# Mictronics/readsb-protobuf

Measured on AMD Instinct MI355X. Metric: IQ Msamples/s, 2.4 MSPS UC8, Mode S demodulation (CRC-valid msgs/s alongside), higher is better.
Workload: dtype int32 (u8 IQ -> u16 magnitude -> int32 correlators, 24-bit CRC)

## Files before the change

readsb-protobuf_amd/csrc/msd_kernels.hip:

```cpp
#include <hip/hip_runtime.h>

#include <cstdlib>

#include "msd_internal.h"
#include "msd_dc_chain_asm.h"
#include "msd_kernels.h"

#ifndef MSD_ARENA_NT
#define MSD_ARENA_NT 1
#endif
#if MSD_ARENA_NT
#define MSD_ARENA_STORE(v, p) __builtin_nontemporal_store((v), (p))
#else
#define MSD_ARENA_STORE(v, p) (*(p) = (v))
#endif
typedef uint32_t msd_v4u __attribute__((ext_vector_type(4)));
__device__ __forceinline__ void arena_store16(const uint4 v, uint4 *p)
{
#if MSD_ARENA_NT
    msd_v4u x = {v.x, v.y, v.z, v.w};
    __builtin_nontemporal_store(x, reinterpret_cast<msd_v4u *>(p));
#else
    *p = v;
#endif
}
#ifndef MSD_AC_PRIO
#define MSD_AC_PRIO 2
#endif
#ifndef MSD_SLICER_SIGN
#define MSD_SLICER_SIGN 1
#endif
#ifndef MSD_TESTS_SWZ
#define MSD_TESTS_SWZ 1
#endif
#ifndef MSD_PRIO_CONV
#define MSD_PRIO_CONV 0
#endif
#ifndef MSD_TESTS_PRE_PLANE
#define MSD_TESTS_PRE_PLANE 1
#endif
#ifndef MSD_PRIO_GATHER
#define MSD_PRIO_GATHER MSD_PRIO_CONV
#endif
#ifndef MSD_PRIO_TESTS
#define MSD_PRIO_TESTS 1
#endif
#ifndef MSD_PRIO_CAND
#define MSD_PRIO_CAND 2
#endif
#ifndef MSD_PRIO_STEPB
#define MSD_PRIO_STEPB 3
#endif
#include "msd_emit_impl.h"
#include "msd_pred_impl.h"
#include "msd_mag_impl.h"

#pragma clang fp contract(off)

#ifdef MSD_KERNEL_TIMING
__device__ unsigned long long g_msd_tlast_dummy;
__device__ __forceinline__ uint32_t msd_cycles()
{
    return (uint32_t)__builtin_readcyclecounter();
}
#define TDECL uint32_t tacc_[12] = {0}; uint32_t tlast_ = msd_cycles();
#define TCOARSE(k) (MSD_KERNEL_TIMING + 0 != 2 || (k) == 0 || (k) == 2 || (k) == 9)
#define TMARK(k) if (TCOARSE(k)) { const uint32_t n_ = msd_cycles(); tacc_[k] += n_ - tlast_; tlast_ = n_; }
#define TMARKF(k) if (MSD_KERNEL_TIMING + 0 != 2) { const uint32_t n_ = msd_cycles(); tacc[k] += n_ - *tlast; *tlast = n_; }
#define TFLUSH if (P.timers && (threadIdx.x & 63) == 0) { for (int k_ = 0; k_ < 12; ++k_) atomicAdd(&P.timers[k_], (unsigned long long)tacc_[k_]); }
#else
#define TDECL
#define TMARK(k)
#define TMARKF(k)
#define TFLUSH
#endif

namespace {

constexpr int WAVES = MSD_SCAN_WAVES;
constexpr int NT = MSD_SCAN_THREADS;
constexpr int WT_MAX = MSD_TILE;
constexpr int FRONT = MSD_HALO_FRONT;
__host__ __device__ constexpr int tile_runs(int fmt)
{
    return (fmt == MSD_FMT_SC16 || fmt == MSD_FMT_SC16Q11) ? 1 : WT_MAX / 1024;
}
constexpr int HC = 64;
constexpr int SC = 64;
constexpr int LUT_STRIDE = MSD_LUT_STRIDE;

static_assert(WT_MAX == 1024 || WT_MAX == 2048 || WT_MAX == 4096, "each lane scans one, two or four runs of 16 consecutive positions");
static_assert(WT_MAX <= 8192, "a position inside a tile has 13 bits in the hit and slot words");
static_assert(FRONT % 8 == 0, "whole load groups");
static_assert(MSD_CHUNK_SAMPLES % WT_MAX == 0, "a tile never straddles two buffers");

constexpr int OFF_SYN = 0;
constexpr int OFF_SL = OFF_SYN + MSD_SYNH_WORDS * 4;
constexpr int OFF_WGC = OFF_SL + MSD_SLICER_WORDS * 4;
constexpr int OFF_WAVE = (OFF_WGC + WAVES * 16 + 15) & ~15;
constexpr int W_MAGS = 0;
constexpr int W_HITS = W_MAGS + (FRONT + WT_MAX + 8) * 2;
constexpr int W_TRYL = W_HITS + HC * 4;
constexpr int W_SIDX = W_TRYL + HC * 5 * 2;
constexpr int W_SMETA = W_SIDX + HC * 8 * 2;
constexpr int W_SMSG = W_SMETA + SC * 4;
constexpr int W_SCRC = W_SMSG + SC * 16;
constexpr int W_SRES = W_SCRC + SC * 4;
constexpr int W_SQOFF = W_SRES + SC * 8;
constexpr int W_BYTES = W_SQOFF + SC * 4;
constexpr int OFF_LUT = OFF_WAVE + WAVES * W_BYTES;
constexpr int LDS_COMMON = OFF_LUT;
constexpr int LDS_UC8 = OFF_LUT + (MSD_LUT_GLOBAL ? 0 : 128 * LUT_STRIDE * 2);
static_assert(OFF_WAVE % 16 == 0 && W_SMSG % 16 == 0 && W_BYTES % 16 == 0 && OFF_LUT % 16 == 0 && W_SIDX % 4 == 0,
              "LDS carve offsets must stay aligned");
static_assert(LDS_UC8 <= 160 * 1024, "one workgroup per CU: 160 KiB of LDS");


template <int FMT>
struct RawGroup {
    static constexpr int WORDS = (FMT == MSD_FMT_SC16 || FMT == MSD_FMT_SC16Q11) ? 8 : 4;
    uint32_t w[WORDS];
};

template <int FMT>
__device__ __forceinline__ uint32_t fetch_group(const MsdScanParams &P, int64_t n, RawGroup<FMT> &r)
{
    constexpr int BPS = RawGroup<FMT>::WORDS / 2;
    const int64_t rel = n - (int64_t)P.batch_first;
    const int64_t left = (int64_t)P.nsamples - rel;
    const uint8_t *src = reinterpret_cast<const uint8_t *>(P.lut);
    uint32_t valid = 0;
    if (rel < 0) {
        if (P.have_prev && rel >= -(int64_t)FRONT) {
            src = P.prev_tail + (rel + FRONT) * BPS;
            valid = 0xffu;
        }
    } else if (left >= 8) {
        src = P.iq + rel * BPS;
        valid = 0xffu;
    } else if (left > 0) {
        src = P.ragged;
        valid = (1u << (int)left) - 1u;
    }
    const uint4 a = *reinterpret_cast<const uint4 *>(src);
    r.w[0] = a.x; r.w[1] = a.y; r.w[2] = a.z; r.w[3] = a.w;
    if (BPS == 4) {
        const uint4 b = *reinterpret_cast<const uint4 *>(src + 16);
        r.w[4 % RawGroup<FMT>::WORDS] = b.x; r.w[5 % RawGroup<FMT>::WORDS] = b.y;
        r.w[6 % RawGroup<FMT>::WORDS] = b.z; r.w[7 % RawGroup<FMT>::WORDS] = b.w;
    }
    return valid;
}

template <int FMT>
__device__ __forceinline__ uint32_t fetch_lookbehind(const MsdScanParams &P, uint64_t pos, int lane, RawGroup<FMT> &r)
{
    constexpr int BPS = RawGroup<FMT>::WORDS / 2;
    if (pos % MSD_CHUNK_SAMPLES != 0)
        return fetch_group<FMT>(P, (int64_t)(P.batch_first + pos) - FRONT + 8 * lane, r);
    const uint32_t slot = P.group_lb[pos / MSD_CHUNK_SAMPLES];
    const bool have = slot != MSD_GROUP_NO_TAIL;
    const uint8_t *src = have ? P.group_tails + ((size_t)slot * FRONT + 8u * (uint32_t)lane) * BPS
                              : reinterpret_cast<const uint8_t *>(P.lut);
    const uint4 a = *reinterpret_cast<const uint4 *>(src);
    r.w[0] = a.x; r.w[1] = a.y; r.w[2] = a.z; r.w[3] = a.w;
    if (BPS == 4) {
        const uint4 b = *reinterpret_cast<const uint4 *>(src + 16);
        r.w[4 % RawGroup<FMT>::WORDS] = b.x; r.w[5 % RawGroup<FMT>::WORDS] = b.y;
        r.w[6 % RawGroup<FMT>::WORDS] = b.z; r.w[7 % RawGroup<FMT>::WORDS] = b.w;
    }
    return have ? 0xffu : 0u;
}

template <int FMT, bool MASK = true ,
          bool SCAN_TABLE = false >
__device__ __forceinline__ void convert_group(const RawGroup<FMT> &r, uint32_t valid, const uint16_t *lut,
                                              uint32_t (&mg)[8])
{
    if (FMT == MSD_FMT_UC8) {
#pragma unroll
        for (int k = 0; k < 4; ++k) {
            const uint32_t w = r.w[k];
            const uint32_t top = w & 0x80808080u;
            const uint32_t keep = top - (top >> 7);
            const uint32_t f = (w ^ ~keep) & 0x7f7f7f7fu;
            if constexpr (SCAN_TABLE) {
                const unsigned char *tab = reinterpret_cast<const unsigned char *>(lut + MSD_LUT_SCAN_OFFSET);
                uint32_t x = f, t, o0, o1;
                if (MSD_LUT_SCAN_SWZ_BITS) {
                    constexpr uint32_t SM = ((1u << MSD_LUT_SCAN_SWZ_BITS) - 1u) << MSD_LUT_SCAN_SWZ_SHIFT;
                    uint32_t r;
                    asm("v_lshrrev_b32 %0, %1, %2" : "=v"(r) : "n"(8 - MSD_LUT_SCAN_SWZ_SHIFT), "v"(f));
                    asm("v_and_b32 %0, %1, %2" : "=v"(r) : "n"(SM | (SM << 16)), "v"(r));
                    asm("v_xor_b32 %0, %1, %2" : "=v"(x) : "v"(f), "v"(r));
                }
                asm("v_add_u32 %0, %1, %1" : "=v"(t) : "v"(x));
                asm("v_and_b32 %0, 0x1fffe, %1" : "=v"(o0) : "v"(t));
                asm("v_lshrrev_b32 %0, 16, %1" : "=v"(o1) : "v"(t));
                mg[2 * k] = *reinterpret_cast<const uint16_t *>(tab + o0);
                mg[2 * k + 1] = *reinterpret_cast<const uint16_t *>(tab + o1);
                continue;
            }
            mg[2 * k] = lut[((f >> 8) & 0xffu) * LUT_STRIDE + (f & 0xffu)];
            mg[2 * k + 1] = lut[(f >> 24) * LUT_STRIDE + ((f >> 16) & 0xffu)];
        }
    } else if (FMT == MSD_FMT_MAG16) {
#pragma unroll
        for (int k = 0; k < 8; ++k)
            mg[k] = (r.w[k >> 1] >> (16 * (k & 1))) & 0xffffu;
    } else {
        const float inv = (FMT == MSD_FMT_SC16) ? (1.0f / 32768.0f) : (1.0f / 2048.0f);
#pragma unroll
        for (int k = 0; k < 8; ++k) {
            const uint32_t w = r.w[k % RawGroup<FMT>::WORDS];
            mg[k] = mag_from_s16((int)(int16_t)(w & 0xffffu), (int)(int16_t)(w >> 16), inv);
        }
    }
    if (MASK && valid != 0xffu) {
#pragma unroll
        for (int k = 0; k < 8; ++k)
            if (!((valid >> k) & 1u))
                mg[k] = 0;
    }
}

__device__ __forceinline__ void mask_group(uint32_t valid, uint32_t (&mg)[8])
{
    if (valid != 0xffu) {
#pragma unroll
        for (int k = 0; k < 8; ++k)
            if (!((valid >> k) & 1u))
                mg[k] = 0;
    }
}

__device__ __forceinline__ uint4 pack8(const uint32_t (&mg)[8])
{
    uint4 p;
    p.x = mg[0] | (mg[1] << 16);
    p.y = mg[2] | (mg[3] << 16);
    p.z = mg[4] | (mg[5] << 16);
    p.w = mg[6] | (mg[7] << 16);
    return p;
}


__device__ __forceinline__ uint32_t pk_shr5(uint32_t pair)
{
    typedef unsigned short us2 __attribute__((ext_vector_type(2)));
    return __builtin_bit_cast(uint32_t, __builtin_bit_cast(us2, pair) >> (unsigned short)5);
}

__device__ __forceinline__ unsigned long long power_sum(uint32_t mod, uint32_t top)
{
    const unsigned long long low = (unsigned long long)top << 10;
    return low + (uint32_t)(mod - (uint32_t)low);
}

__device__ __forceinline__ uint32_t dot2u(uint32_t pair, uint32_t weights, uint32_t acc)
{
    typedef unsigned short us2 __attribute__((ext_vector_type(2)));
    return __builtin_amdgcn_udot2(__builtin_bit_cast(us2, pair), __builtin_bit_cast(us2, weights), acc, false);
}

__device__ __forceinline__ uint32_t bytes_for_df(uint32_t df)
{
    const uint32_t short_set = (1u << 0) | (1u << 4) | (1u << 5) | (1u << 11);
    const uint32_t long_set = (1u << 16) | (1u << 17) | (1u << 18) | (1u << 20) | (1u << 21) | (1u << 24);
    if ((short_set >> df) & 1u)
        return 7;
    if ((long_set >> df) & 1u)
        return 14;
    return 1;
}

__device__ __forceinline__ uint32_t wave_incl_scan(uint32_t v)
{
    uint32_t x = v;
    x += (uint32_t)__builtin_amdgcn_update_dpp(0, (int)x, 0x111, 0xf, 0xf, false);
    x += (uint32_t)__builtin_amdgcn_update_dpp(0, (int)x, 0x112, 0xf, 0xf, false);
    x += (uint32_t)__builtin_amdgcn_update_dpp(0, (int)x, 0x114, 0xf, 0xf, false);
    x += (uint32_t)__builtin_amdgcn_update_dpp(0, (int)x, 0x118, 0xf, 0xf, false);
    x += (uint32_t)__builtin_amdgcn_update_dpp(0, (int)x, 0x142, 0xa, 0xf, false);
    x += (uint32_t)__builtin_amdgcn_update_dpp(0, (int)x, 0x143, 0xc, 0xf, false);
    return x;
}

__device__ __forceinline__ uint32_t wave_last(uint32_t v)
{
    return (uint32_t)__builtin_amdgcn_readlane((int)v, 63);
}

__device__ __forceinline__ void wave_lds_sync()
{
    __builtin_amdgcn_fence(__ATOMIC_RELEASE, "wavefront");
    __builtin_amdgcn_wave_barrier();
    __builtin_amdgcn_fence(__ATOMIC_ACQUIRE, "wavefront");
}

#define MSD_PUSH(PLANE, MASK) asm("v_addc_co_u32 %0, vcc, %0, %0, %1" : "+v"(PLANE) : "s"(MASK) : "vcc")

template <int EXTRA>
__device__ __forceinline__ void group_load(const unsigned char *const (&a)[5], uint32_t (&m)[5][4])
{
    typedef __attribute__((address_space(3))) const volatile uint16_t lds_sample;
#pragma unroll
    for (int c = 0; c < 5; ++c) {
        lds_sample *p = (lds_sample *)(a[c] + EXTRA);
        m[c][0] = p[0];
        m[c][1] = p[1];
        m[c][2] = p[2];
        m[c][3] = c == 4 ? p[3] : 0u;
    }
}

__device__ __forceinline__ int mad24(int a, int b, int c)
{
    int d;
    asm("v_mad_i32_i24 %0, %1, %2, %3" : "=v"(d) : "v"(a), "v"(b), "v"(c));
    return d;
}

__device__ __forceinline__ uint32_t group_code(const uint32_t (&m)[5][4])
{
    uint32_t code = 0;
#if MSD_SLICER_SIGN
    const int c6 = -6, c5 = 5, c14 = -14, c16 = -16, cm5 = -5, c20 = 20, c7 = -7, c11 = -11, c18 = 18, c4 = -4, c15 = -15;
    const int y4 = mad24((int)m[4][2], c20, mad24((int)m[4][1], c15, mad24((int)m[4][0], c4, -(int)m[4][3])));
    code = __builtin_amdgcn_alignbit(code, (uint32_t)y4, 31);
    const int y1 = mad24((int)m[1][0], c14, mad24((int)m[1][1], c5, (int)(m[1][2] * 9u)));
    code = __builtin_amdgcn_alignbit(code, (uint32_t)y1, 31);
    const int y3 = mad24((int)m[3][2], c18, mad24((int)m[3][1], c11, (int)m[3][0] * c7));
    code = __builtin_amdgcn_alignbit(code, (uint32_t)y3, 31);
    const int y0 = mad24((int)m[0][1], c5, mad24((int)m[0][0], c6, (int)m[0][2]));
    code = __builtin_amdgcn_alignbit(code, (uint32_t)y0, 31);
    const int y2 = mad24((int)m[2][2], c20, mad24((int)m[2][1], cm5, (int)m[2][0] * c16));
    code = __builtin_amdgcn_alignbit(code, (uint32_t)y2, 31);
#else
    const uint64_t b4 = __ballot(4u * m[4][0] + 15u * m[4][1] + m[4][3] > 20u * m[4][2]);
    MSD_PUSH(code, b4);
    const uint64_t b1 = __ballot(14u * m[1][0] > 5u * m[1][1] + 9u * m[1][2]);
    MSD_PUSH(code, b1);
    const uint64_t b3 = __ballot(7u * m[3][0] + 11u * m[3][1] > 18u * m[3][2]);
    MSD_PUSH(code, b3);
    const uint64_t b0 = __ballot(18u * m[0][0] > 15u * m[0][1] + 3u * m[0][2]);
    MSD_PUSH(code, b0);
    const uint64_t b2 = __ballot(16u * m[2][0] + 5u * m[2][1] > 20u * m[2][2]);
    MSD_PUSH(code, b2);
#endif
    return code;
}

__device__ __forceinline__ uint32_t phase_rot(uint32_t q)
{
    return (0x31420u >> (4u * q)) & 7u;
}

__device__ __forceinline__ uint32_t group_bits(uint32_t code, uint32_t rot)
{
    return ((code | (code << 5)) >> rot) & 31u;
}

template <int EXTRA>
__device__ __forceinline__ uint32_t group_verdicts(const unsigned char *const (&a)[5], uint32_t rot)
{
    uint32_t m[5][4];
    group_load<EXTRA>(a, m);
    return group_bits(group_code(m), rot);
}

struct WaveCtx {
    unsigned char *w;
    const uint32_t *syn;
    const uint32_t *sl;
    int lane;
};

template <bool FIX2, bool GROUP = false>
__device__ __forceinline__ bool candidate_round(const MsdScanParams &P, const WaveCtx &X, uint32_t nh, uint64_t tile_pos0,
                                                msd_hit *hit_out, uint32_t hits_room, msd_try *my_tries,
                                                uint32_t &tcur, uint32_t try_base ,
                                                uint32_t nfix
#ifdef MSD_KERNEL_TIMING
                                                , uint32_t *tacc, uint32_t *tlast
#endif
                                                )
{
    const int lane = X.lane;
    const unsigned char *mbytes = X.w + W_MAGS;
    const uint32_t *hitl = reinterpret_cast<const uint32_t *>(X.w + W_HITS);
    uint16_t *tryl = reinterpret_cast<uint16_t *>(X.w + W_TRYL);
    uint16_t *sidx = reinterpret_cast<uint16_t *>(X.w + W_SIDX);
    uint32_t *smeta = reinterpret_cast<uint32_t *>(X.w + W_SMETA);
    uint32_t *smsg32 = reinterpret_cast<uint32_t *>(X.w + W_SMSG);
    uint32_t *scrc = reinterpret_cast<uint32_t *>(X.w + W_SCRC);
    uint32_t *sres = reinterpret_cast<uint32_t *>(X.w + W_SRES);
    uint32_t *sqoff = reinterpret_cast<uint32_t *>(X.w + W_SQOFF);

    uint32_t my_hit = 0, my_m = 0;
    {
        *reinterpret_cast<uint4 *>(sidx + 8 * lane) = make_uint4(~0u, ~0u, ~0u, ~0u);
        if ((uint32_t)lane < nh) {
            my_hit = hitl[lane];
            my_m = my_hit >> 13;
        }
    }
    const uint32_t nt = 2u * (my_m & 1u) + (my_m & 2u) + ((my_m >> 2) & 1u);
    const uint32_t tincl = wave_incl_scan(nt);
    const uint32_t ntry = wave_last(tincl);
    {
        uint32_t k = tincl - nt;
        if (my_m & 1u) {
            tryl[k] = (uint16_t)lane;
            tryl[k + 1] = (uint16_t)(lane | (1 << 8));
            k += 2;
        }
        if (my_m & 2u) {
            tryl[k] = (uint16_t)(lane | (2 << 8));
            tryl[k + 1] = (uint16_t)(lane | (3 << 8));
            k += 2;
        }
        if (my_m & 4u)
            tryl[k] = (uint16_t)(lane | (4 << 8));
    }
    wave_lds_sync();

    uint32_t ns = 0, nl = 0;
    for (uint32_t i0 = 0; i0 < ntry; i0 += 64) {
        const uint32_t i = i0 + (uint32_t)lane;
        const bool act = i < ntry;
        const uint32_t e = act ? tryl[i] : 0u;
        const uint32_t h = e & 0xffu, q = e >> 8;
        const uint32_t pos = hitl[h] & 0x1fffu;
        const uint32_t qoff = X.sl[MSD_SL_QOFF + q];
        const unsigned char *base = mbytes + 2u * pos + 4u;
        const unsigned char *a[5];
#pragma unroll
        for (int c = 0; c < 5; ++c)
            a[c] = base + ((qoff >> (6 * c)) & 63u);
        const uint32_t df = group_verdicts<0>(a, phase_rot(q));
        const uint32_t nb = bytes_for_df(df);
        const bool is_s = act && nb == 7, is_l = act && nb == 14;
        const uint64_t bs = __ballot(is_s), bl = __ballot(is_l);
        const uint32_t rs = __builtin_amdgcn_mbcnt_hi((uint32_t)(bs >> 32), __builtin_amdgcn_mbcnt_lo((uint32_t)bs, 0u));
        const uint32_t rl = __builtin_amdgcn_mbcnt_hi((uint32_t)(bl >> 32), __builtin_amdgcn_mbcnt_lo((uint32_t)bl, 0u));
        const uint32_t u = is_s ? ns + rs : (uint32_t)(SC - 1) - (nl + rl);
        ns += (uint32_t)__popcll(bs);
        nl += (uint32_t)__popcll(bl);
        if (ns + nl > (uint32_t)SC)
            return false;
        if (is_s || is_l) {
            smeta[u] = pos | (q << 13) | (nb << 16) | (h << 20);
            *reinterpret_cast<uint4 *>(smsg32 + 4u * u) = make_uint4(df << 27, 0u, 0u, 0u);
            scrc[u] = X.sl[(is_l ? MSD_SL_GLONG : MSD_SL_GSHORT) + df];
            sqoff[u] = qoff;
            sidx[h * 8u + q] = (uint16_t)u;
        }
    }
    wave_lds_sync();
    TMARKF(4)

    if (!(P.debug_flags & 4)) {
        if (MSD_PRIO_STEPB != MSD_PRIO_CAND)
            __builtin_amdgcn_s_setprio(MSD_PRIO_STEPB);
        constexpr uint32_t NG = MSD_SLICER_NG, IS = (11 + NG - 1) / NG, IL = (22 + NG - 1) / NG;
        constexpr uint32_t VB = 5 * NG;
        constexpr uint32_t LAST_S = 51 - VB * (IS - 1), LAST_L = 107 - VB * (IL - 1);
        constexpr uint32_t MASK_S = ((1u << LAST_S) - 1u) << (VB - LAST_S), MASK_L = ((1u << LAST_L) - 1u) << (VB - LAST_L);
        const uint32_t short_items = IS * ns, nitems = short_items + IL * nl;
        for (uint32_t i0 = 0; i0 < nitems; i0 += 64) {
            const uint32_t i = i0 + (uint32_t)lane;
            const bool act = i < nitems;
            const bool lng = i >= short_items;
            const uint32_t j = act ? (lng ? i - short_items : i) : 0u;
            const uint32_t t = (j * (lng ? (65536u + IL - 1) / IL : (65536u + IS - 1) / IS)) >> 16;
            const uint32_t it = j - t * (lng ? IL : IS);
            const uint32_t u = lng ? (uint32_t)(SC - 1) - t : t;
            const uint32_t me = smeta[u];
            const uint32_t qoff = sqoff[u];
            const uint32_t pos = me & (uint32_t)(WT_MAX - 1), q = (me >> 13) & 7u;
            const uint32_t g1 = NG * it + 1u;
            const unsigned char *base = mbytes + 2u * pos + 4u + 24u * g1;
            const unsigned char *a[5];
#pragma unroll
            for (int c = 0; c < 5; ++c)
                a[c] = base + ((qoff >> (6 * c)) & 63u);
            const uint32_t rot = phase_rot(q);
            uint32_t v[NG];
            v[0] = group_verdicts<0>(a, rot);
            if (NG > 1) v[1 % NG] = group_verdicts<24>(a, rot);
            if (NG > 2) v[2 % NG] = group_verdicts<48>(a, rot);
            if (NG > 3) v[3 % NG] = group_verdicts<72>(a, rot);
            if (NG > 4) v[4 % NG] = group_verdicts<96>(a, rot);
            uint32_t val = 0;
#pragma unroll
            for (uint32_t c = 0; c < NG; ++c)
                val |= v[c] << (5u * (NG - 1u - c));
            if (it == (lng ? IL - 1u : IS - 1u))
                val &= lng ? MASK_L : MASK_S;
            if (act) {
                const uint32_t *gt = X.sl + (lng ? MSD_SL_GLONG : MSD_SL_GSHORT) + 32u * g1;
                uint32_t syn = 0;
#pragma unroll
                for (uint32_t c = 0; c < NG; ++c) {
                    const uint32_t e = (val >> (5u * (NG - 1u - c))) & 31u;
                    if (NG * IL <= 24u && NG * IS <= 12u)
                        syn ^= gt[32u * c + e];
                    else if (e)
                        syn ^= gt[32u * c + e];
                }
                atomicXor(&scrc[u], syn);
                const uint32_t n0 = 5u * g1, s = n0 & 31u, top = val << (32u - VB);
                atomicOr(&smsg32[4u * u + (n0 >> 5)], top >> s);
                if (s > 32u - VB)
                    atomicOr(&smsg32[4u * u + (n0 >> 5) + 1u], __builtin_amdgcn_alignbit(top, 0u, s));
            }
        }
        if (MSD_PRIO_STEPB != MSD_PRIO_CAND)
            __builtin_amdgcn_s_setprio(MSD_PRIO_CAND);
    }
    wave_lds_sync();
    TMARKF(5)

    if ((uint32_t)lane < ns || (uint32_t)lane >= (uint32_t)SC - nl) {
        const uint32_t u = (uint32_t)lane;
        const uint32_t me = smeta[u];
        const uint4 m4 = *reinterpret_cast<const uint4 *>(smsg32 + 4u * u);
        const uint32_t crc = scrc[u];
        const uint32_t df = m4.x >> 27, aa = m4.x & 0xffffffu;
        bool alive = (m4.x | m4.y | m4.z | m4.w) != 0;
        uint32_t addr = crc, errbit = 0xffu, errbit2 = 0xffu;
        if (alive && (df == 11 || df == 17 || df == 18)) {
            addr = aa;
            const uint32_t syndrome = (df == 11) ? (crc & 0xffff80u) : crc;
            if (syndrome != 0) {
                alive = false;
                if (FIX2 && (!GROUP || nfix == 2)) {
                    const uint64_t *tab = (df == 11) ? P.fix2_56 : P.fix2_112;
                    const uint32_t lg = (df == 11) ? P.fix2_lg56 : P.fix2_lg112;
                    uint32_t slot = MSD_FIX2_HASH(syndrome, lg);
                    for (;;) {
                        const uint64_t e = tab[slot];
                        if (e == ~0ull)
                            break;
                        if (((uint32_t)e & 0xffffffu) == syndrome) {
                            errbit = (uint32_t)(e >> 32) & 0xffu;
                            errbit2 = (uint32_t)(e >> 40) & 0xffu;
                            alive = !(df == 11 && errbit2 != 0xffu);
                            break;
                        }
                        slot = (slot + 1) & ((1u << lg) - 1u);
                    }
                } else {
                    if (GROUP ? nfix != 0 : P.nsyn112 != 0) {
                        const uint32_t bkt = (df == 11) ? (syndrome * P.synh_mul56) >> (32u - MSD_SYNH_LG56)
                                                        : (4u << MSD_SYNH_LG56) / 4u + ((syndrome * P.synh_mul112) >> (32u - MSD_SYNH_LG112));
                        const uint4 e4 = *reinterpret_cast<const uint4 *>(X.syn + 4u * bkt);
                        const uint32_t e[4] = {e4.x, e4.y, e4.z, e4.w};
#pragma unroll
                        for (int j = 0; j < 4; ++j)
                            if ((e[j] & 0xffffffu) == syndrome) {
                                errbit = e[j] >> 24;
                                alive = true;
                            }
                    }
                }
                if (alive && errbit >= 8 && errbit <= 31)
                    addr ^= 1u << (31 - errbit);
                if (alive && errbit2 >= 8 && errbit2 <= 31)
                    addr ^= 1u << (31 - errbit2);
            }
        }
        const uint32_t q = (me >> 13) & 7u, h = me >> 20;
        if (alive && crc == 0 && (df == 17 || df == 11) && P.pred)
            msd_pred_note(P.pred, P.pred_gen, aa, (uint32_t)(tile_pos0 / MSD_CHUNK_SAMPLES));
        if (alive) {
            *reinterpret_cast<uint4 *>(smsg32 + 4u * u) =
                make_uint4(__builtin_bswap32(m4.x), __builtin_bswap32(m4.y), __builtin_bswap32(m4.z),
                           (__builtin_bswap32(m4.w) & 0xffffu) | ((4u + q) << 16) | (errbit << 24));
            sres[2 * u] = addr;
            sres[2 * u + 1] = crc | (errbit2 << 24);
        } else {
            sidx[h * 8u + q] = 0xffffu;
        }
    }
    wave_lds_sync();
    TMARKF(6)

    uint32_t u5[5], nlive = 0;
#pragma unroll
    for (int q = 0; q < 5; ++q) {
        u5[q] = (uint32_t)lane < nh ? (uint32_t)sidx[lane * 8 + q] : 0xffffu;
        nlive += u5[q] != 0xffffu ? 1u : 0u;
    }
    const uint32_t lincl = wave_incl_scan(nlive);
    const uint32_t ntry_round = wave_last(lincl);
    if ((uint32_t)lane < nh && (uint32_t)lane < hits_room) {
        const uint32_t pos = my_hit & 0x1fffu;
        msd_hit rec = (tile_pos0 + pos) | ((msd_hit)my_m << 28) | ((msd_hit)nlive << 31);
        if (nlive)
            rec |= (msd_hit)(try_base + tcur + lincl - nlive) << 34;
        hit_out[lane] = rec;
    }
    wave_lds_sync();
    {
        uint32_t k = lincl - nlive;
#pragma unroll
        for (int q = 0; q < 5; ++q)
            if (u5[q] != 0xffffu)
                sidx[k++] = (uint16_t)(u5[q] | ((uint32_t)lane << 9));
    }
    wave_lds_sync();
    for (uint32_t e0 = 0; e0 < ntry_round; e0 += 32u) {
        const uint32_t e = e0 + ((uint32_t)lane >> 1);
        const bool mine = e < ntry_round && tcur + e < P.tcap;
        const uint32_t ent = mine ? (uint32_t)sidx[e] : 0u;
        const uint32_t u = ent & 0x1ffu;
        const uint32_t pos = (uint32_t)__shfl((int)(my_hit & 0x1fffu), (int)(ent >> 9), 64);
        if (mine) {
            uint4 *dst = reinterpret_cast<uint4 *>(my_tries + tcur + e);
            const uint4 m16 = *reinterpret_cast<const uint4 *>(smsg32 + 4u * u);
            if (!(lane & 1)) {
                arena_store16(m16, &dst[0]);
            } else {
                const uint32_t cw = sres[2 * u + 1];
                arena_store16(make_uint4(sres[2 * u], cw & 0xffffffu, (uint32_t)(tile_pos0 + pos),
                                         (cw >> 24) | ((m16.x & 0xffu) << 8) | (m16.w & 0xffff0000u)),
                              &dst[1]);
            }
        }
    }
    tcur += ntry_round;
    wave_lds_sync();
    TMARKF(7)
    return true;
}

template <int FMT>
__device__ inline void msd_emit_slice(const MsdEmitJob &J, const uint16_t *lut_g, uint32_t w, int lane, unsigned char *lds,
                                      bool dbg_no_store = false);

template <int FMT, bool FIX2, bool EMIT, bool GROUP>
__device__ __forceinline__ void scan_region(const MsdScanParams &P, const WaveCtx &X, const uint16_t *lut,
                                            uint32_t region, uint32_t tile_lo, uint32_t tile_hi, uint32_t &hits_total,
                                            uint32_t &tries_total)
{
    constexpr int NH = tile_runs(FMT), WT = 1024 * NH;
    constexpr bool SCAN_LUT = MSD_LUT_SCAN256 && MSD_LUT_GLOBAL;
    constexpr int GPT = WT / 8 / 64;
    const int lane = X.lane;
    uint16_t *mags = reinterpret_cast<uint16_t *>(X.w + W_MAGS);
    uint32_t *hitl = reinterpret_cast<uint32_t *>(X.w + W_HITS);
    const uint64_t batch_end = P.batch_first + P.nsamples;
    msd_hit *const my_hits = P.hits + (size_t)region * P.hcap;
    msd_try *const my_tries = P.tries + (size_t)region * P.tcap;
    const uint32_t try_base = P.regions_per_buffer ? region * P.tcap : 0u;
    uint32_t hcur = 0, tcur = 0;

    uint32_t sum_level = 0;
    uint32_t pw_mod = 0, pw_top = 0, sum_tiles = 0, sum_tile0 = tile_lo;
    uint64_t sum_chunk = (uint64_t)tile_lo * WT / MSD_CHUNK_SAMPLES;
    unsigned long long acc_level = 0, acc_power = 0;
    auto flush_sums = [&]() {
        if (P.chunk_sums && P.tile_sums) {
            if (sum_tiles) {
                const unsigned long long sp = power_sum(pw_mod, pw_top);
                const uint32_t tl = wave_last(wave_incl_scan((uint32_t)sum_level));
                const uint32_t tlo = wave_last(wave_incl_scan((uint32_t)sp & 0xffffffu));
                const uint32_t thi = wave_last(wave_incl_scan((uint32_t)(sp >> 24)));
                const unsigned long long tp = ((unsigned long long)thi << 24) + tlo;
                acc_level += tl;
                acc_power += tp;
                if (lane == 0) {
                    P.tile_sums[2 * sum_tile0] = (float)tl * (1.0f / 65535.0f);
                    P.tile_sums[2 * sum_tile0 + 1] = (float)tp * (1.0f / (65535.0f * 65535.0f));
                }
            }
        } else if (P.chunk_sums) {
            const unsigned long long spl = power_sum(pw_mod, pw_top);
            const unsigned long long sl = wave_last(wave_incl_scan((uint32_t)sum_level));
            const unsigned long long sp = (unsigned long long)wave_last(wave_incl_scan((uint32_t)spl & 0xffffffu)) +
                                          ((unsigned long long)wave_last(wave_incl_scan((uint32_t)(spl >> 24))) << 24);
            if (lane == 0 && (sl | sp)) {
                atomicAdd(reinterpret_cast<unsigned long long *>(&P.chunk_sums[2 * sum_chunk]), sl);
                atomicAdd(reinterpret_cast<unsigned long long *>(&P.chunk_sums[2 * sum_chunk + 1]), sp);
            }
        }
        sum_level = 0;
        pw_mod = 0;
        pw_top = 0;
        sum_tiles = 0;
    };
    auto flush_chunk = [&]() {
        if (P.chunk_sums && P.tile_sums && lane == 0 && (acc_level | acc_power)) {
            atomicAdd(reinterpret_cast<unsigned long long *>(&P.chunk_sums[2 * sum_chunk]), acc_level);
            atomicAdd(reinterpret_cast<unsigned long long *>(&P.chunk_sums[2 * sum_chunk + 1]), acc_power);
        }
        acc_level = 0;
        acc_power = 0;
    };

    {
        const uint64_t a0 = P.batch_first + (uint64_t)tile_lo * WT;
        if (lane < FRONT / 8) {
            RawGroup<FMT> r;
            uint32_t valid;
            if constexpr (GROUP)
                valid = fetch_lookbehind<FMT>(P, (uint64_t)tile_lo * WT, lane, r);
            else
                valid = fetch_group<FMT>(P, (int64_t)a0 - FRONT + 8 * lane, r);
            uint32_t mg[8];
            convert_group<FMT, true, SCAN_LUT>(r, valid, lut, mg);
            *reinterpret_cast<uint4 *>(mags + 8 * lane) = pack8(mg);
        }
    }
    RawGroup<FMT> cur[GPT], nxt[GPT];
    uint32_t cur_valid[GPT], nxt_valid[GPT];
    {
        const uint64_t a0 = P.batch_first + (uint64_t)tile_lo * WT;
#pragma unroll
        for (int k = 0; k < GPT; ++k) {
            cur_valid[k] = fetch_group<FMT>(P, (int64_t)a0 + 8 * (lane + 64 * k), cur[k]);
            nxt_valid[k] = 0;
            nxt[k] = cur[k];
        }
    }
    auto fetch_tile = [&](uint32_t ti) {
        const int64_t rel = (int64_t)((uint64_t)ti * WT);
        if ((uint64_t)rel + WT <= (P.nsamples & ~7ull)) {
            constexpr int BPS = RawGroup<FMT>::WORDS / 2;
#pragma unroll
            for (int k = 0; k < GPT; ++k) {
                const uint8_t *src = P.iq + (rel + 8 * (lane + 64 * k)) * BPS;
                const uint4 a = *reinterpret_cast<const uint4 *>(src);
                nxt[k].w[0] = a.x; nxt[k].w[1] = a.y; nxt[k].w[2] = a.z; nxt[k].w[3] = a.w;
                if (BPS == 4) {
                    const uint4 b = *reinterpret_cast<const uint4 *>(src + 16);
                    nxt[k].w[4 % RawGroup<FMT>::WORDS] = b.x; nxt[k].w[5 % RawGroup<FMT>::WORDS] = b.y;
                    nxt[k].w[6 % RawGroup<FMT>::WORDS] = b.z; nxt[k].w[7 % RawGroup<FMT>::WORDS] = b.w;
                }
                nxt_valid[k] = 0xffu;
            }
        } else {
#pragma unroll
            for (int k = 0; k < GPT; ++k)
                nxt_valid[k] = fetch_group<FMT>(P, (int64_t)P.batch_first + rel + 8 * (lane + 64 * k), nxt[k]);
        }
    };

    const uint32_t emit_at = EMIT && P.emit.nbuffers && region / P.emit.stride < P.emit.nbuffers ? tile_lo + region % (tile_hi - tile_lo) : 0xffffffffu;

    TDECL
    for (uint32_t tile = tile_lo; tile < tile_hi; ++tile) {
        const uint64_t tile_pos0 = (uint64_t)tile * WT;
        TMARK(8)
        uint32_t gopt = 0;
        if constexpr (GROUP)
            gopt = P.group_opt[tile_pos0 / MSD_CHUNK_SAMPLES];
        const uint64_t a0 = P.batch_first + tile_pos0;

        {
            const uint64_t c = tile_pos0 / MSD_CHUNK_SAMPLES;
            if (c != sum_chunk || sum_tiles == (P.tile_sums ? 1u : 16u / NH)) {
                flush_sums();
                if (c != sum_chunk)
                    flush_chunk();
                sum_chunk = c;
                sum_tile0 = tile;
            }
            ++sum_tiles;
        }
        uint32_t mgs[GPT][8], mg_valid[GPT];
        if (MSD_PRIO_GATHER != MSD_PRIO_CONV)
            __builtin_amdgcn_s_setprio(MSD_PRIO_GATHER);
#pragma unroll
        for (int k = 0; k < GPT; ++k) {
            convert_group<FMT, false, SCAN_LUT>(cur[k], cur_valid[k], lut, mgs[k]);
            mg_valid[k] = cur_valid[k];
        }
        if (MSD_PRIO_GATHER != MSD_PRIO_CONV)
            __builtin_amdgcn_s_setprio(MSD_PRIO_CONV);
#pragma unroll
        for (int k = 0; k < GPT; ++k) {
            uint32_t(&mg)[8] = mgs[k];
            mask_group(mg_valid[k], mg);
            const uint4 packed = pack8(mg);
            *reinterpret_cast<uint4 *>(mags + FRONT + 8 * (lane + 64 * k)) = packed;
            if (P.mag_out)
                arena_store16(packed, reinterpret_cast<uint4 *>(P.mag_out + tile_pos0 + 8u * (uint32_t)(lane + 64 * k)));
            const uint32_t pk[4] = {packed.x, packed.y, packed.z, packed.w};
#pragma unroll
            for (int i = 0; i < 4; ++i) {
                sum_level = dot2u(pk[i], 0x00010001u, sum_level);
                pw_mod = dot2u(pk[i], pk[i], pw_mod);
                const uint32_t top = pk_shr5(pk[i]);
                pw_top = dot2u(top, top, pw_top);
            }
        }
        wave_lds_sync();
        TMARK(0)

        if (EMIT && tile == emit_at && !(P.debug_flags & 128))
            msd_emit_slice<FMT>(P.emit, P.lut, region, lane, X.w + W_HITS, (P.debug_flags & 64) != 0);

        if (tile + 1 < tile_hi)
            fetch_tile(tile + 1);

        TMARK(1)
        if (!(P.debug_flags & 2)) {
            if (MSD_PRIO_TESTS != MSD_PRIO_CONV)
                __builtin_amdgcn_s_setprio(MSD_PRIO_TESTS);
            uint32_t pl0[NH], pl1[NH], pl2[NH], any[NH], cnt[NH], rank0[NH];
            uint32_t H = 0;
#pragma unroll
            for (int h = 0; h < NH; ++h) {
                uint32_t v[20];
                {
                    const uint4 *src = reinterpret_cast<const uint4 *>(mags + 1024 * h + 16 * lane);
#if MSD_TESTS_SWZ
                    const bool odd_first = (lane & 16) != 0;
                    const int k0 = odd_first ? 1 : 0, k2 = odd_first ? 3 : 2;
                    const uint4 r0 = src[k0], r1 = src[k0 ^ 1], r2 = src[k2], r3 = src[k2 ^ 1], r4 = src[4];
                    const uint4 c0 = odd_first ? r1 : r0, c1 = odd_first ? r0 : r1, c2 = odd_first ? r3 : r2, c3 = odd_first ? r2 : r3;
                    v[0] = c0.x; v[1] = c0.y; v[2] = c0.z; v[3] = c0.w;
                    v[4] = c1.x; v[5] = c1.y; v[6] = c1.z; v[7] = c1.w;
                    v[8] = c2.x; v[9] = c2.y; v[10] = c2.z; v[11] = c2.w;
                    v[12] = c3.x; v[13] = c3.y; v[14] = c3.z; v[15] = c3.w;
                    v[16] = r4.x; v[17] = r4.y; v[18] = r4.z; v[19] = r4.w;
#else
#pragma unroll
                    for (int k = 0; k < 5; ++k) {
                        const uint4 q = src[k];
                        v[4 * k] = q.x; v[4 * k + 1] = q.y; v[4 * k + 2] = q.z; v[4 * k + 3] = q.w;
                    }
#endif
                }
#if MSD_TESTS_V2
                int sm[40];
#pragma unroll
                for (int k = 0; k < 20; ++k) {
                    asm("v_and_b32 %0, 0xffff, %1" : "=v"(sm[2 * k]) : "v"(v[k]));
                    asm("v_lshrrev_b32 %0, 16, %1" : "=v"(sm[2 * k + 1]) : "v"(v[k]));
                }
                uint32_t p0 = 0, p1 = 0, p2 = 0;
#if MSD_TESTS_PRE_PLANE
                uint32_t ppre = 0;
#endif
                const int thr = GROUP ? (int)(gopt & 0xffffu) : P.threshold, m32 = -32;
#pragma unroll
                for (int q = 0; q < 16; ++q) {
#define PA(d) (sm[q + 2 + (d)])
                    const int pre = (PA(7) - PA(1)) & (PA(14) - PA(12)) & (PA(15) - PA(12));
                    const int base_noise = PA(5) + PA(8) + PA(16) + PA(17) + PA(18);
                    int refm;
                    asm("v_mad_u32_u24 %0, %1, %2, %3" : "=v"(refm) : "v"(base_noise), "v"(thr), "v"(m32));
                    refm >>= 5;
                    const int diff_2_3 = PA(2) - PA(3), diff_10_11 = PA(10) - PA(11);
                    const int b = refm - (PA(1) + PA(4) + PA(12));
                    const int r1 = b + diff_2_3 - PA(9);
#if MSD_TESTS_PRE_PLANE
                    const int g0 = r1 + diff_10_11, g1 = r1 - diff_10_11;
                    const int g2 = b - diff_2_3 - diff_2_3 - diff_10_11;
                    ppre = __builtin_amdgcn_alignbit(ppre, (uint32_t)pre, 31);
#else
                    const int g0 = pre & (r1 + diff_10_11), g1 = pre & (r1 - diff_10_11);
                    const int g2 = pre & (b - diff_2_3 - diff_2_3 - diff_10_11);
#endif
#undef PA
                    p0 = __builtin_amdgcn_alignbit(p0, (uint32_t)g0, 31);
                    p1 = __builtin_amdgcn_alignbit(p1, (uint32_t)g1, 31);
                    p2 = __builtin_amdgcn_alignbit(p2, (uint32_t)g2, 31);
                }
#if MSD_TESTS_PRE_PLANE
                p0 &= ppre;
                p1 &= ppre;
                p2 &= ppre;
#endif
#else
                int sm[40];
#pragma unroll
                for (int k = 0; k < 20; ++k) {
                    sm[2 * k] = (int)(v[k] & 0xffffu);
                    sm[2 * k + 1] = (int)(v[k] >> 16);
                }
                uint32_t p0 = 0, p1 = 0, p2 = 0;
#pragma unroll
                for (int q = 0; q < 16; ++q) {
#define PA(d) (sm[q + 2 + (d)])
                    const uint64_t pre = __ballot(PA(1) > PA(7)) & __ballot(PA(12) > PA(14)) & __ballot(PA(12) > PA(15));
                    const uint32_t base_noise = (uint32_t)(PA(5) + PA(8) + PA(16) + PA(17) + PA(18));
                    const int ref_level = (int)(__umul24(base_noise, GROUP ? gopt & 0xffffu : (uint32_t)P.threshold) >> 5);
                    const int diff_2_3 = PA(2) - PA(3);
                    const int sum_1_4 = PA(1) + PA(4);
                    const int diff_10_11 = PA(10) - PA(11);
                    const int common3456 = sum_1_4 - diff_2_3 + PA(9) + PA(12);
                    const uint64_t f0 = pre & __ballot(common3456 - diff_10_11 >= ref_level);
                    const uint64_t f1 = pre & __ballot(common3456 + diff_10_11 >= ref_level);
                    const uint64_t f2 = pre & __ballot(sum_1_4 + 2 * diff_2_3 + diff_10_11 + PA(12) >= ref_level);
#undef PA
                    MSD_PUSH(p0, f0);
                    MSD_PUSH(p1, f1);
                    MSD_PUSH(p2, f2);
                }
#endif
                {
                    const uint64_t first = a0 + 1024ull * h + 16ull * lane;
                    if (first + 16 > batch_end) {
                        const int keep = first >= batch_end ? 0 : (int)(batch_end - first);
                        const uint32_t km = keep ? ~((1u << (16 - keep)) - 1u) : 0u;
                        p0 &= km;
                        p1 &= km;
                        p2 &= km;
                    }
                }
                pl0[h] = p0;
                pl1[h] = p1;
                pl2[h] = p2;
                any[h] = p0 | p1 | p2;

                cnt[h] = (uint32_t)__popc(any[h]);
                const uint32_t incl = wave_incl_scan(cnt[h]);
                rank0[h] = H + incl - cnt[h];
                H += wave_last(incl);
            }

            TMARK(2)
            if (MSD_PRIO_CAND != MSD_PRIO_TESTS)
                __builtin_amdgcn_s_setprio(MSD_PRIO_CAND);
            if (!(P.debug_flags & 1) && H) {
                uint32_t r0 = 0;
                bool fill = true;
                uint32_t nh = (H < (uint32_t)HC) ? H : (uint32_t)HC;
                while (r0 < H) {
                    if (fill) {
#pragma unroll
                        for (int h = 0; h < NH; ++h) {
                            if (cnt[h] && rank0[h] < r0 + HC && rank0[h] + cnt[h] > r0) {
                                uint32_t x = any[h], r = rank0[h];
                                while (x) {
                                    const int bit = 31 - __clz((int)x);
                                    x &= ~(1u << bit);
                                    if (r >= r0 && r < r0 + HC) {
                                        const uint32_t m = ((pl0[h] >> bit) & 1u) | (((pl1[h] >> bit) & 1u) << 1) |
                                                           (((pl2[h] >> bit) & 1u) << 2);
                                        hitl[r - r0] = (uint32_t)(1024 * h + 16 * lane + (15 - bit)) | (m << 13);
                                    }
                                    ++r;
                                }
                            }
                        }
                        wave_lds_sync();
                    }
                    const uint32_t out0 = hcur + r0;
                    const uint32_t room = out0 < P.hcap ? P.hcap - out0 : 0u;
                    TMARK(3)
                    if (!candidate_round<FIX2, GROUP>(P, X, nh, tile_pos0, my_hits + out0, room, my_tries, tcur, try_base,
                                                      gopt >> 16
#ifdef MSD_KERNEL_TIMING
                                               , tacc_, &tlast_
#endif
                                               )) {
                        nh = (nh + 1) / 2;
                        fill = false;
                        wave_lds_sync();
                    } else {
                        r0 += nh;
                        nh = (H - r0 < (uint32_t)HC) ? (H - r0) : (uint32_t)HC;
                        fill = true;
                    }
                }
            }
            hcur += H;
            if (MSD_PRIO_CAND != MSD_PRIO_CONV)
                __builtin_amdgcn_s_setprio(MSD_PRIO_CONV);
        }
        TMARK(9)

        if (GROUP && tile + 1 < tile_hi && (tile_pos0 + WT) % MSD_CHUNK_SAMPLES == 0) {
            uint4 lb = make_uint4(0, 0, 0, 0);
            if (lane < FRONT / 8) {
                RawGroup<FMT> r;
                const uint32_t valid = fetch_lookbehind<FMT>(P, tile_pos0 + WT, lane, r);
                uint32_t mg[8];
                convert_group<FMT, true, SCAN_LUT>(r, valid, lut, mg);
                lb = pack8(mg);
            }
            wave_lds_sync();
            if (lane < FRONT / 8)
                *reinterpret_cast<uint4 *>(mags + 8 * lane) = lb;
        } else {
            uint4 carry = make_uint4(0, 0, 0, 0);
            if (lane < FRONT / 8)
                carry = *reinterpret_cast<const uint4 *>(mags + WT + 8 * lane);
            wave_lds_sync();
            if (lane < FRONT / 8)
                *reinterpret_cast<uint4 *>(mags + 8 * lane) = carry;
        }
#pragma unroll
        for (int k = 0; k < GPT; ++k) {
            cur[k] = nxt[k];
            cur_valid[k] = nxt_valid[k];
        }
    }
    TMARK(8)
    TFLUSH
    flush_sums();
    flush_chunk();
    hits_total = hcur;
    tries_total = tcur;
}

template <int FMT, bool FIX2 ,
          bool EMIT ,
          bool GROUP = false >
#ifndef MSD_SCAN_OCC
#define MSD_SCAN_OCC ((MSD_SCAN_WAVES * MSD_SCAN_WGS_PER_CU + 3) / 4)
#endif
__global__ void __launch_bounds__(NT, MSD_SCAN_OCC) msd_scan_kernel(const MsdScanParams P)
{
    extern __shared__ __attribute__((aligned(16))) unsigned char smem[];
    uint32_t *syn = reinterpret_cast<uint32_t *>(smem + OFF_SYN);
    uint32_t *sl = reinterpret_cast<uint32_t *>(smem + OFF_SL);
    uint32_t *wgc = reinterpret_cast<uint32_t *>(smem + OFF_WGC);
    uint16_t *lds_lut = reinterpret_cast<uint16_t *>(smem + OFF_LUT);
    const uint16_t *lut = MSD_LUT_GLOBAL ? P.lut : lds_lut;

    const int tid = threadIdx.x, lane = tid & 63, wave = __builtin_amdgcn_readfirstlane(tid >> 6);

    for (int i = tid; i < (int)MSD_SYNH_WORDS; i += NT)
        syn[i] = P.synhash[i];
    for (int i = tid; i < (int)MSD_SLICER_WORDS; i += NT)
        sl[i] = P.slicer[i];
    if (FMT == MSD_FMT_UC8 && !MSD_LUT_GLOBAL) {
        const uint4 *g = reinterpret_cast<const uint4 *>(P.lut);
        uint4 *l = reinterpret_cast<uint4 *>(lds_lut);
        for (int i = tid; i < 128 * LUT_STRIDE * 2 / 16; i += NT)
            l[i] = g[i];
    }
    __syncthreads();

    const uint32_t region = blockIdx.x * WAVES + (uint32_t)wave;
    uint32_t tile_lo, tile_hi;
    if (P.regions_per_buffer) {
        constexpr uint32_t TPB = MSD_CHUNK_SAMPLES / (1024u * tile_runs(FMT));
        const uint32_t b = region / P.regions_per_buffer, piece = region - b * P.regions_per_buffer;
        tile_lo = b * TPB + piece * P.tiles_per_region;
        tile_hi = tile_lo + P.tiles_per_region;
        if (tile_hi > (b + 1) * TPB)
            tile_hi = (b + 1) * TPB;
        if (tile_lo > tile_hi)
            tile_lo = tile_hi;
        if (region == 0 && P.tail_words)
            for (uint32_t i = (uint32_t)lane; i < P.tail_words; i += 64)
                P.tail_dst[i] = P.tail_src[i];
    } else {
        tile_lo = region * P.tiles_per_wg;
        tile_hi = tile_lo + P.tiles_per_wg;
    }
    if (tile_hi > P.ntiles)
        tile_hi = P.ntiles;
    uint32_t nhits = 0, ntries = 0;
    if (tile_lo < tile_hi) {
        WaveCtx X;
        X.w = smem + OFF_WAVE + wave * W_BYTES;
        X.syn = syn;
        X.sl = sl;
        X.lane = lane;
        scan_region<FMT, FIX2, EMIT, GROUP>(P, X, lut, region, tile_lo, tile_hi, nhits, ntries);
    } else if (EMIT && P.emit.nbuffers && region / P.emit.stride < P.emit.nbuffers && !(P.debug_flags & 128)) {
        msd_emit_slice<FMT>(P.emit, P.lut, region, lane, smem + OFF_WAVE + wave * W_BYTES + W_HITS, (P.debug_flags & 64) != 0);
    }
    if (lane == 0) {
        wgc[4 * wave] = nhits;
        wgc[4 * wave + 1] = ntries;
        wgc[4 * wave + 2] = (nhits > P.hcap || ntries > P.tcap) ? 1u : 0u;
    }
    __syncthreads();
    if (tid < WAVES) {
        msd_region_counts c = {};
        uint32_t hb = 0, tb = 0, ovf = 0;
        for (int i = 0; i < WAVES; ++i) {
            if (i == tid) {
                c.hbase = hb;
                c.tbase = tb;
            }
            hb += wgc[4 * i];
            tb += wgc[4 * i + 1];
            ovf |= wgc[4 * i + 2];
        }
        c.nhits = wgc[4 * tid];
        c.ntries = wgc[4 * tid + 1];
        c.overflow = wgc[4 * tid + 2];
        P.counts[blockIdx.x * WAVES + tid] = c;
        if (tid == 0) {
            msd_wg_totals t = {hb, tb, ovf, 0};
            P.wg_totals[blockIdx.x] = t;
            if (ovf && P.overflow)
                atomicOr(P.overflow, 1ull);
        }
    }
}

__global__ void __launch_bounds__(256) msd_gather_kernel(const msd_region_counts *counts, const msd_wg_totals *wgt,
                                                         const msd_hit *hits, const msd_try *tries, uint32_t hcap,
                                                         uint32_t tcap, msd_hit *dense_hits, uint64_t dense_hcap,
                                                         msd_try *dense_tries, uint64_t dense_tcap, uint64_t *totals,
                                                         uint64_t *sums, uint32_t nbuffers, uint64_t *h_totals,
                                                         uint64_t *h_sums, uint4 *wipe, uint32_t wipe_n,
                                                         const uint32_t *tail_src, uint32_t *tail_dst,
                                                         uint32_t tail_words, uint32_t region_len, uint32_t *buf_first,
                                                         uint32_t try_abs )
{
    __shared__ unsigned long long ph[4], pt[4];
    __shared__ uint32_t povf[4];
    const uint32_t w = blockIdx.x, nreg = gridDim.x, tid = threadIdx.x;
    const uint32_t my_wg = w / WAVES, nswg = (nreg + WAVES - 1) / WAVES;
    unsigned long long h = 0, t = 0;
    uint32_t ovf = 0;
    const bool last = w + 1 == nreg;
    for (uint32_t i = tid; i < (last ? nswg : my_wg); i += 256) {
        const msd_wg_totals c = wgt[i];
        if (i < my_wg) {
            h += c.nhits;
            t += c.ntries;
        }
        ovf |= c.overflow;
    }
#pragma unroll
    for (int d = 32; d > 0; d >>= 1) {
        h += __shfl_down(h, d, 64);
        t += __shfl_down(t, d, 64);
        ovf |= __shfl_down(ovf, d, 64);
    }
    if ((tid & 63) == 0) {
        ph[tid >> 6] = h;
        pt[tid >> 6] = t;
        povf[tid >> 6] = ovf;
    }
    __syncthreads();
    const msd_region_counts mine = counts[w];
    const uint64_t ho = ph[0] + ph[1] + ph[2] + ph[3] + mine.hbase, to = pt[0] + pt[1] + pt[2] + pt[3] + mine.tbase;
    const uint32_t nh = mine.nhits < hcap ? mine.nhits : hcap;
    const uint32_t nt = mine.ntries < tcap ? mine.ntries : tcap;
    if (last) {
        if (tid == 0) {
            const uint64_t ah = ho + mine.nhits, at = to + mine.ntries;
            const uint64_t o = (povf[0] | povf[1] | povf[2] | povf[3]) ? 1 : 0;
            totals[0] = ah;
            totals[1] = at;
            totals[2] = o;
            if (h_totals) {
                h_totals[0] = ah;
                h_totals[1] = at;
                h_totals[2] = o;
            }
        }
        if (h_sums)
            for (uint32_t i = tid; i < 2 * nbuffers; i += 256) {
                h_sums[i] = sums[i];
                sums[i] = 0;
            }
    }
    if (w == 0)
        for (uint32_t i = tid; i < tail_words; i += 256)
            tail_dst[i] = tail_src[i];
    for (uint32_t i = w * blockDim.x + tid; i < wipe_n; i += nreg * blockDim.x)
        wipe[i] = make_uint4(~0u, ~0u, ~0u, ~0u);
    const msd_hit *hs = hits + (size_t)w * hcap;
    if (buf_first && tid < 64) {
        const uint64_t p0 = (uint64_t)w * region_len, p1 = last ? ~0ull : p0 + region_len;
        for (uint64_t bb = (p0 + MSD_CHUNK_SAMPLES - 1) / MSD_CHUNK_SAMPLES; bb <= nbuffers && bb * MSD_CHUNK_SAMPLES < p1; ++bb) {
            const uint64_t want = bb * MSD_CHUNK_SAMPLES;
            uint32_t lo = 0, hi = nh;
            while (lo < hi) {
                const uint32_t step = (hi - lo + 63) / 64, p = lo + tid * step;
                const bool below = p < hi && MSD_HIT_POS(hs[p]) < want;
                const uint32_t k = (uint32_t)__popcll(__ballot(below));
                if (k == 0) {
                    hi = lo;
                } else {
                    const uint32_t nhi = lo + k * step;
                    lo = lo + (k - 1) * step + 1;
                    if (nhi < hi)
                        hi = nhi;
                }
            }
            if (tid == 0)
                buf_first[bb] = (uint32_t)(ho + lo < 0xffffffffull ? ho + lo : 0xffffffffull);
        }
    }
    for (uint32_t i = tid; i < nh; i += blockDim.x) {
        msd_hit hr = hs[i];
        if (MSD_HIT_NLIVE(hr))
            hr = (hr & ((1ull << 34) - 1)) | ((MSD_HIT_TRY(hr) - (try_abs ? (uint64_t)w * tcap : 0ull) + to) << 34);
        if (ho + i < dense_hcap)
            dense_hits[ho + i] = hr;
    }
    const uint4 *ts = reinterpret_cast<const uint4 *>(tries + (size_t)w * tcap);
    uint4 *td = reinterpret_cast<uint4 *>(dense_tries);
    for (uint32_t i = tid; i < 2 * nt; i += blockDim.x)
        if (to + (i >> 1) < dense_tcap)
            td[2 * to + i] = ts[i];
}


__global__ void __launch_bounds__(256) msd_offsets_kernel(const msd_wg_counts *counts, uint32_t nwg,
                                                          uint64_t *offsets ,
                                                          uint64_t *totals , uint64_t *sums,
                                                          uint32_t nbuffers, uint64_t *h_totals, uint64_t *h_sums)
{
    __shared__ unsigned long long sh[256], st[256];
    __shared__ uint32_t ovf;
    const int tid = threadIdx.x;
    if (tid == 0)
        ovf = 0;
    __syncthreads();
    const uint32_t per = (nwg + 255) / 256;
    unsigned long long h = 0, t = 0;
    for (uint32_t i = tid * per; i < (tid + 1) * per && i < nwg; ++i) {
        h += counts[i].nhits;
        t += counts[i].ntries;
        if (counts[i].overflow)
            atomicOr(&ovf, 1u);
    }
    sh[tid] = h;
    st[tid] = t;
    __syncthreads();
    if (tid == 0) {
        unsigned long long ah = 0, at = 0;
        for (int i = 0; i < 256; ++i) {
            const unsigned long long x = sh[i], y = st[i];
            sh[i] = ah;
            st[i] = at;
            ah += x;
            at += y;
        }
        totals[0] = ah;
        totals[1] = at;
        totals[2] = ovf;
        if (h_totals) {
            h_totals[0] = ah;
            h_totals[1] = at;
            h_totals[2] = ovf;
        }
    }
    if (h_sums)
        for (uint32_t i = tid; i < 2 * nbuffers; i += 256) {
            h_sums[i] = sums[i];
            sums[i] = 0;
        }
    __syncthreads();
    h = sh[tid];
    t = st[tid];
    for (uint32_t i = tid * per; i < (tid + 1) * per && i < nwg; ++i) {
        offsets[2 * i] = h;
        offsets[2 * i + 1] = t;
        h += counts[i].nhits;
        t += counts[i].ntries;
    }
}


template <int FMT>
__device__ __forceinline__ uint32_t stream_mag(const MsdScanParams &P, int64_t n, const uint16_t *lut_g)
{
    MsdSampleSource S;
    S.iq = P.iq;
    S.prev_tail = P.prev_tail;
    S.have_prev = P.have_prev;
    S.batch_first = P.batch_first;
    S.nsamples = P.nsamples;
    return msd_stream_mag<FMT>(S, n, lut_g);
}

template <int FMT>
__device__ inline void msd_emit_slice(const MsdEmitJob &J, const uint16_t *lut_g, uint32_t w, int lane, unsigned char *lds,
                                      bool dbg_no_store)
{
    const uint32_t b = w / J.stride, slice = w % J.stride;
    const uint64_t ovf = J.totals[2], ac_ovf = J.ac ? J.ac_totals[2] : 0;
    const uint32_t nm = J.nmsgs[b], na_all = J.ac ? J.nac[b] : 0u;
    uint32_t o;
    if (J.rec_off) {
        o = J.rec_off[b];
    } else {
        uint32_t mine = 0;
        for (uint32_t i = (uint32_t)lane; i < b; i += 64)
            mine += J.nmsgs[i] + (J.ac ? J.nac[i] : 0u);
        o = wave_last(wave_incl_scan(mine));
    }
    if (ovf || ac_ovf)
        return;
    const uint64_t sample_ts = J.ts[2 * b], sys_ts = J.ts[2 * b + 1];
    const uint32_t base = b * MSD_CHUNK_SAMPLES;
    const msd_acc *acc = J.acc + (size_t)b * MSD_RB_MSG_CAP;
    constexpr uint32_t ROUND = 32;
    msd_wire *rec = reinterpret_cast<msd_wire *>(lds);
    static_assert(sizeof(msd_wire) % 8 == 0 && ROUND * sizeof(msd_wire) <= W_BYTES - W_HITS, "the records of a round fit the candidate scratch");
    auto flush = [&](uint32_t first, uint32_t n) {
        __builtin_amdgcn_fence(__ATOMIC_RELEASE, "wavefront");
        __builtin_amdgcn_wave_barrier();
        if (first < J.cap && !dbg_no_store) {
            n = min(n, J.cap - first);
            unsigned long long *d = reinterpret_cast<unsigned long long *>(J.dense + first);
// ... 1975 lines not shown
```

Measured before the change: 385,400.

## Make next-tile prefetch branch-free and retire it before candidate phase

The next-tile prefetch is restructured so every group always issues one uniform load, with per-lane pointer selection (real input, ragged tail, or dummy LUT) replacing the divergent full/partial branch. Validity masks are packed into one word instead of per-group arrays. The cur/nxt rotation moves before the candidate phase and uses an asm register pin, so the prefetched data is consumed and its registers freed earlier. An explicit vmcnt wait is added after the emit slice. The aim is to cut branching and register pressure around the prefetch while keeping loads overlapped with the tests. The trade-off is that loads are issued even for the last tile, and the earlier wait may stall on outstanding loads.

```diff
diff --git a/readsb-protobuf_amd/csrc/msd_kernels.hip b/readsb-protobuf_amd/csrc/msd_kernels.hip
--- a/readsb-protobuf_amd/csrc/msd_kernels.hip
+++ b/readsb-protobuf_amd/csrc/msd_kernels.hip
@@ -150,6 +150,17 @@
         r.w[6 % RawGroup<FMT>::WORDS] = b.z; r.w[7 % RawGroup<FMT>::WORDS] = b.w;
     }
     return valid;
+}
+
+constexpr int WAIT_VM0 = 0x0f70;
+
+template <int FMT>
+__device__ __forceinline__ void hold_group(RawGroup<FMT> &r)
+{
+    if constexpr (RawGroup<FMT>::WORDS == 4)
+        asm volatile("" : "+v"(r.w[0]), "+v"(r.w[1]), "+v"(r.w[2]), "+v"(r.w[3]));
+    else
+        asm volatile("" : "+v"(r.w[0]), "+v"(r.w[1]), "+v"(r.w[2]), "+v"(r.w[3]), "+v"(r.w[4]), "+v"(r.w[5]), "+v"(r.w[6]), "+v"(r.w[7]));
 }
 
 template <int FMT>
@@ -715,36 +726,52 @@
         }
     }
     RawGroup<FMT> cur[GPT], nxt[GPT];
-    uint32_t cur_valid[GPT], nxt_valid[GPT];
+    uint32_t cur_valid = 0, nxt_valid = 0;
+    static_assert(GPT <= 4, "a byte of the mask word per group");
     {
         const uint64_t a0 = P.batch_first + (uint64_t)tile_lo * WT;
 #pragma unroll
         for (int k = 0; k < GPT; ++k) {
-            cur_valid[k] = fetch_group<FMT>(P, (int64_t)a0 + 8 * (lane + 64 * k), cur[k]);
-            nxt_valid[k] = 0;
+            cur_valid |= fetch_group<FMT>(P, (int64_t)a0 + 8 * (lane + 64 * k), cur[k]) << (8 * k);
             nxt[k] = cur[k];
         }
     }
-    auto fetch_tile = [&](uint32_t ti) {
-        const int64_t rel = (int64_t)((uint64_t)ti * WT);
-        if ((uint64_t)rel + WT <= (P.nsamples & ~7ull)) {
-            constexpr int BPS = RawGroup<FMT>::WORDS / 2;
+    auto fetch_tile = [&](uint32_t ti, bool exists) {
+        constexpr int BPS = RawGroup<FMT>::WORDS / 2;
+        const uint64_t rel = (uint64_t)ti * WT;
+        const uint8_t *src[GPT];
+#pragma unroll
+        for (int k = 0; k < GPT; ++k)
+            src[k] = P.iq + (rel + 8 * lane) * BPS + 8 * 64 * BPS * k;
+        nxt_valid = 0xffffffffu >> (32 - 8 * GPT);
+        const uint64_t have = exists && rel < P.nsamples ? P.nsamples - rel : 0;
+        if (have < (uint64_t)WT) {
+            nxt_valid = 0;
 #pragma unroll
             for (int k = 0; k < GPT; ++k) {
-                const uint8_t *src = P.iq + (rel + 8 * (lane + 64 * k)) * BPS;
-                const uint4 a = *reinterpret_cast<const uint4 *>(src);
-                nxt[k].w[0] = a.x; nxt[k].w[1] = a.y; nxt[k].w[2] = a.z; nxt[k].w[3] = a.w;
-                if (BPS == 4) {
-                    const uint4 b = *reinterpret_cast<const uint4 *>(src + 16);
-                    nxt[k].w[4 % RawGroup<FMT>::WORDS] = b.x; nxt[k].w[5 % RawGroup<FMT>::WORDS] = b.y;
-                    nxt[k].w[6 % RawGroup<FMT>::WORDS] = b.z; nxt[k].w[7 % RawGroup<FMT>::WORDS] = b.w;
+                const int left = (int)have - 8 * (lane + 64 * k);
+                const uint8_t *s = reinterpret_cast<const uint8_t *>(P.lut);
+                uint32_t v = 0;
+                if (left >= 8) {
+                    s = src[k];
+                    v = 0xffu;
+                } else if (left > 0) {
+                    s = P.ragged;
+                    v = (1u << left) - 1u;
                 }
-                nxt_valid[k] = 0xffu;
-            }
-        } else {
-#pragma unroll
-            for (int k = 0; k < GPT; ++k)
-                nxt_valid[k] = fetch_group<FMT>(P, (int64_t)P.batch_first + rel + 8 * (lane + 64 * k), nxt[k]);
+                src[k] = s;
+                nxt_valid |= v << (8 * k);
+            }
+        }
+#pragma unroll
+        for (int k = 0; k < GPT; ++k) {
+            const uint4 a = *reinterpret_cast<const uint4 *>(src[k]);
+            nxt[k].w[0] = a.x; nxt[k].w[1] = a.y; nxt[k].w[2] = a.z; nxt[k].w[3] = a.w;
+            if (BPS == 4) {
+                const uint4 b = *reinterpret_cast<const uint4 *>(src[k] + 16);
+                nxt[k].w[4 % RawGroup<FMT>::WORDS] = b.x; nxt[k].w[5 % RawGroup<FMT>::WORDS] = b.y;
+                nxt[k].w[6 % RawGroup<FMT>::WORDS] = b.z; nxt[k].w[7 % RawGroup<FMT>::WORDS] = b.w;
+            }
         }
     };
 
@@ -775,8 +802,8 @@
             __builtin_amdgcn_s_setprio(MSD_PRIO_GATHER);
 #pragma unroll
         for (int k = 0; k < GPT; ++k) {
-            convert_group<FMT, false, SCAN_LUT>(cur[k], cur_valid[k], lut, mgs[k]);
-            mg_valid[k] = cur_valid[k];
+            mg_valid[k] = (cur_valid >> (8 * k)) & 0xffu;
+            convert_group<FMT, false, SCAN_LUT>(cur[k], mg_valid[k], lut, mgs[k]);
         }
         if (MSD_PRIO_GATHER != MSD_PRIO_CONV)
             __builtin_amdgcn_s_setprio(MSD_PRIO_CONV);
@@ -800,25 +827,28 @@
         wave_lds_sync();
         TMARK(0)
 
-        if (EMIT && tile == emit_at && !(P.debug_flags & 128))
+        if (EMIT && tile == emit_at && !(P.debug_flags & 128)) {
             msd_emit_slice<FMT>(P.emit, P.lut, region, lane, X.w + W_HITS, (P.debug_flags & 64) != 0);
-
-        if (tile + 1 < tile_hi)
-            fetch_tile(tile + 1);
+            __builtin_amdgcn_s_waitcnt(WAIT_VM0);
+        }
+
+        fetch_tile(tile + 1, tile + 1 < tile_hi);
 
         TMARK(1)
+        uint32_t pl0[NH], pl1[NH], pl2[NH], any[NH], cnt[NH], rank0[NH];
+        uint32_t H = 0;
         if (!(P.debug_flags & 2)) {
             if (MSD_PRIO_TESTS != MSD_PRIO_CONV)
                 __builtin_amdgcn_s_setprio(MSD_PRIO_TESTS);
-            uint32_t pl0[NH], pl1[NH], pl2[NH], any[NH], cnt[NH], rank0[NH];
-            uint32_t H = 0;
 #pragma unroll
             for (int h = 0; h < NH; ++h) {
                 uint32_t v[20];
                 {
                     const uint4 *src = reinterpret_cast<const uint4 *>(mags + 1024 * h + 16 * lane);
 #if MSD_TESTS_SWZ
-                    const bool odd_first = (lane & 16) != 0;
+                    int l = lane;
+                    asm volatile("" : "+v"(l));
+                    const bool odd_first = (l & 16) != 0;
                     const int k0 = odd_first ? 1 : 0, k2 = odd_first ? 3 : 2;
                     const uint4 r0 = src[k0], r1 = src[k0 ^ 1], r2 = src[k2], r3 = src[k2 ^ 1], r4 = src[4];
                     const uint4 c0 = odd_first ? r1 : r0, c1 = odd_first ? r0 : r1, c2 = odd_first ? r3 : r2, c3 = odd_first ? r2 : r3;
@@ -923,7 +953,16 @@
                 rank0[h] = H + incl - cnt[h];
                 H += wave_last(incl);
             }
-
+        }
+
+#pragma unroll
+        for (int k = 0; k < GPT; ++k) {
+            hold_group<FMT>(nxt[k]);
+            cur[k] = nxt[k];
+        }
+        cur_valid = nxt_valid;
+
+        if (!(P.debug_flags & 2)) {
             TMARK(2)
             if (MSD_PRIO_CAND != MSD_PRIO_TESTS)
                 __builtin_amdgcn_s_setprio(MSD_PRIO_CAND);
@@ -995,11 +1034,6 @@
             wave_lds_sync();
             if (lane < FRONT / 8)
                 *reinterpret_cast<uint4 *>(mags + 8 * lane) = carry;
-        }
-#pragma unroll
-        for (int k = 0; k < GPT; ++k) {
-            cur[k] = nxt[k];
-            cur_valid[k] = nxt_valid[k];
         }
     }
     TMARK(8)
```

Measured after the change: 392,400 (median of 6 runs). +1.8%, better.
